# PJLab-ADG/nr3d_lib

Hardware: AMD Instinct MI355X
Metric: Mpoints/s LoTD fwd+bwd (16-lvl hash) + Mrays/s march+composite, 1 & 8 GPU (higher is better)
Workload: dtype f32; 1 GPU; configs[1]: 16-level Hash LoTD (gen_ngp_cfg: T=2^19, F=2, 6 Dense + 10 Hash), 2^20 points/GPU, fwd(+dy/dx) + dL/dx + dL/dparam, fp32; points_per_gpu=1048576, n_params=12131648, parallelism=single GPU

## Files before the change

nr3d_lib_amd/csrc/lotd_pair.hip:

```cpp
#include "lotd_device.h"
#include <stdlib.h>


namespace nr3d {
namespace lotd {

constexpr uint32_t kPEpbMax = 8192;
constexpr int kPAccThreads = 1024;
constexpr int kPLdsMax = 2 * (int)kPEpbMax;
constexpr int kPMaxLv = 32;
constexpr uint32_t kPMaxNb = 511;
typedef uint32_t u32x4 __attribute__((ext_vector_type(4)));

struct PairPlan {
	uint32_t qmap[kPMaxLv];
	uint32_t nb[kPMaxLv];
	uint32_t epb[kPMaxLv];
	uint32_t shift[kPMaxLv];
	uint32_t bucket_base[kPMaxLv + 1];
	uint32_t offs_base[kPMaxLv];
	uint32_t n_blk, n_pseudo;
	uint32_t cap;
	uint32_t lg;
	uint32_t sum_log2;
// ... 318 lines not shown
		uint32_t gbits;
		if constexpr (!SECOND) {
			gbits = max(__float_as_uint(g0) & 0x7FFFFFFFu, __float_as_uint(g1) & 0x7FFFFFFFu);
			if (ql == 0 && i < n)
				for (uint32_t e = 0; e < dp.n; ++e) {
					const uint32_t qd = dp.qmap[e];
					if ((int32_t)meta_level_of(md, qd) > max_level) continue;
					gbits = max(gbits, __float_as_uint(g[(int64_t)i * g_sn + (int64_t)(qd * 2) * g_se]) & 0x7FFFFFFFu);
					gbits = max(gbits, __float_as_uint(g[(int64_t)i * g_sn + (int64_t)(qd * 2 + 1) * g_se]) & 0x7FFFFFFFu);
				}
		} else {
			auto bound = [&](const Lvl &Lq, float ga, float gb) {
				const float m = __uint_as_float(max(__float_as_uint(ga) & 0x7FFFFFFFu, __float_as_uint(gb) & 0x7FFFFFFFu)) * 1.5f *
				                ((float)(Lq.res[0] - 2u) * fabsf(vin[0]) + (float)(Lq.res[1] - 2u) * fabsf(vin[1]) + (float)(Lq.res[2] - 2u) * fabsf(vin[2]));
				return __float_as_uint(m) & 0x7FFFFFFFu;
			};
			gbits = bound(L, g0, g1);
			if (ql == 0 && i < n) {
				if (!active) {
#pragma unroll
					for (int d = 0; d < 3; ++d) vin[d] = vin_[(size_t)i * 3 + d];
				}
				for (uint32_t e = 0; e < dp.n; ++e) {
					const uint32_t qd = dp.qmap[e];
					if ((int32_t)meta_level_of(md, qd) > max_level) continue;
					const Lvl Ld = load_level(md, meta_level_of(md, qd));
					gbits = max(gbits, bound(Ld, g[(int64_t)i * g_sn + (int64_t)(qd * 2) * g_se], g[(int64_t)i * g_sn + (int64_t)(qd * 2 + 1) * g_se]));
				}
			}
		}
		pair_gmax<kPBP>(gbits, scan_lds, gmax);
	}
}

__device__ __forceinline__ uint32_t gmax_slots(const uint32_t *__restrict__ slots, uint32_t n_slots, uint32_t *red) {
	uint32_t m = 0;
	for (uint32_t k = threadIdx.x; k < n_slots; k += 1024u) m = max(m, slots[k]);
#pragma unroll
	for (int off = 32; off >= 1; off >>= 1) m = max(m, (uint32_t)__shfl_xor((int)m, off, 64));
	__syncthreads();
	if ((threadIdx.x & 63u) == 0) red[threadIdx.x >> 6] = m;
	__syncthreads();
	m = 0;
#pragma unroll
	for (int k = 0; k < 16; ++k) m = max(m, red[k]);
	__syncthreads();
	return m;
}

__device__ __forceinline__ void pair_plan_block(const PairPlan &plan, const uint32_t *__restrict__ offs_g, uint32_t n_units,
                                                uint32_t *__restrict__ tot, uint32_t *__restrict__ rep,
                                                uint32_t *__restrict__ item_start, uint32_t *__restrict__ ticket, uint32_t bid,
                                                uint32_t nblk, const uint32_t *__restrict__ slots, uint32_t n_slots,
                                                uint32_t *__restrict__ gmax_out, bool empty_one) {
	__shared__ uint64_t red[16];
	__shared__ uint64_t carry_s;
	__shared__ uint32_t last_s;
	const uint32_t lane = threadIdx.x & 63, wave = threadIdx.x >> 6;
	const uint32_t NB = plan.bucket_base[plan.n_pseudo];
	{
		const uint32_t fb = bid * 16 + wave;
		if (fb < NB) {
			uint32_t q = 0;
			while (q + 1 < plan.n_pseudo && plan.bucket_base[q + 1] <= fb) ++q;
			const uint32_t *ob0 = offs_g + plan.offs_base[q] + (size_t)(fb - plan.bucket_base[q]) * plan.n_blk;
			const uint32_t *ob1 = ob0 + plan.n_blk;
			uint32_t sum = 0;
			for (uint32_t blk = lane; blk < plan.n_blk; blk += 64) sum += ob1[blk] - ob0[blk];
#pragma unroll
			for (int off = 32; off >= 1; off >>= 1) sum += __shfl_xor(sum, off, 64);
			if (lane == 0) __hip_atomic_store(tot + fb, sum, __ATOMIC_RELAXED, __HIP_MEMORY_SCOPE_AGENT);
		}
	}
	__syncthreads();
	if (threadIdx.x == 0) {
		__builtin_amdgcn_fence(__ATOMIC_RELEASE, "agent");
		asm volatile("s_waitcnt vmcnt(0)" ::: "memory");
		last_s = (atomicAdd(ticket, 1u) == nblk - 1u) ? 1u : 0u;
		__builtin_amdgcn_fence(__ATOMIC_ACQUIRE, "agent");
	}
	__syncthreads();
	if (!last_s) return;
	if (slots) {
		const uint32_t gb = gmax_slots(slots, n_slots, reinterpret_cast<uint32_t *>(red));
		if (threadIdx.x == 0) gmax_out[0] = gb;
	}
	auto ld_tot = [&](uint32_t fb) { return (uint64_t)__hip_atomic_load(tot + fb, __ATOMIC_RELAXED, __HIP_MEMORY_SCOPE_AGENT); };
	uint64_t part = 0;
	for (uint32_t fb = threadIdx.x; fb < NB; fb += 1024) part += ld_tot(fb);
#pragma unroll
	for (int off = 32; off >= 1; off >>= 1) part += __shfl_xor(part, off, 64);
	if (lane == 0) red[wave] = part;
	__syncthreads();
	uint64_t total = 0;
#pragma unroll
	for (int w = 0; w < 16; ++w) total += red[w];
	const uint64_t unit = total / n_units > 0 ? total / n_units : 1;
	if (threadIdx.x == 0) carry_s = 0;
	__syncthreads();
	for (uint32_t base = 0; base < NB; base += 1024) {
		const uint32_t fb = base + threadIdx.x;
		uint32_t r = 0;
		if (fb < NB) {
			const uint64_t t = ld_tot(fb);
			r = t == 0 ? (empty_one ? 1u : 0u) : (uint32_t)((t + unit / 2) / unit);
			if (t != 0 && r < 1) r = 1;
			if (r > plan.n_blk) r = plan.n_blk;
			rep[fb] = r;
		}
		uint64_t inc = r;
#pragma unroll
		for (int off = 1; off < 64; off <<= 1) { const uint64_t t2 = __shfl_up(inc, off, 64); if ((int)lane >= off) inc += t2; }
		__syncthreads();
		if (lane == 63) red[wave] = inc;
		__syncthreads();
		uint64_t woff = 0, tsum = 0;
#pragma unroll
		for (int w = 0; w < 16; ++w) { if (w < (int)wave) woff += red[w]; tsum += red[w]; }
		const uint64_t c = carry_s;
		if (fb < NB) item_start[fb] = (uint32_t)(c + woff + inc - r);
		__syncthreads();
		if (threadIdx.x == 0) carry_s = c + tsum;
		__syncthreads();
	}
	if (threadIdx.x == 0) item_start[NB] = (uint32_t)carry_s;
}
__global__ __launch_bounds__(1024) void k_pair_plan(PairPlan plan, const uint32_t *__restrict__ offs_g, uint32_t n_units,
                                                    uint32_t *__restrict__ tot, uint32_t *__restrict__ rep,
                                                    uint32_t *__restrict__ item_start, uint32_t *__restrict__ ticket,
                                                    const uint32_t *__restrict__ slots, uint32_t n_slots, uint32_t *__restrict__ gmax_out,
                                                    uint32_t empty_one) {
	pair_plan_block(plan, offs_g, n_units, tot, rep, item_start, ticket, blockIdx.x, gridDim.x, slots, n_slots, gmax_out, empty_one != 0u);
}

__device__ __forceinline__ float *pair_target(const Lvl &L, uint32_t epb, uint32_t lg, uint32_t foff0, uint32_t b, uint32_t t,
                                              float *__restrict__ dparam, bool out_half = false) {
	const uint32_t f = t >> lg, el = t & ((1u << lg) - 1u);
	const uint64_t entry = (uint64_t)b * epb + el;
	if (el >= epb || entry >= L.size) return nullptr;
	const uint64_t at = L.off + (entry * L.F + foff0 + f);
	return out_half ? reinterpret_cast<float *>(reinterpret_cast<__half *>(dparam) + at) : dparam + at;
}
__device__ __forceinline__ float pair_ld(const float *p, bool out_half) {
	return out_half ? __half2float(*reinterpret_cast<const __half *>(p)) : *p;
}
__device__ __forceinline__ void pair_st(float *p, float v, bool out_half) {
	if (out_half) *reinterpret_cast<__half *>(p) = __float2half(v); else *p = v;
}

struct PairFix { double scale, inv; bool on; };
__device__ __forceinline__ PairFix pair_fix_bits(uint32_t bits, uint32_t sum_log2) {
	PairFix f;
	f.on = bits < 0x7F800000u;
	const int e = max((int)(bits >> 23), 1) - 126;
	const int lim = min(62 - (int)sum_log2, 50 - 6);
	const int sc = max(min(lim - e, 1000), -1000);
	f.scale = __longlong_as_double((long long)(sc + 1023) << 52);
	f.inv = __longlong_as_double((long long)(1023 - sc) << 52);
	return f;
}
__device__ __forceinline__ PairFix pair_fix(const uint32_t *__restrict__ gmax, uint32_t sum_log2) {
	return pair_fix_bits(((cu32_t)gmax)[0], sum_log2);
}
__device__ __forceinline__ unsigned long long to_fix(float v, double scale) {
	const double t = __fma_rn((double)v, scale, 0x1.8p52);
	return (unsigned long long)(__double_as_longlong(t) - 0x4338000000000000LL);
}

__device__ __forceinline__ float pair_replica_sum(const float *__restrict__ part_t, uint32_t R, uint32_t kPLds) {
	float sum = 0.0f;
	uint32_t r0 = 0;
	for (; r0 + 8 <= R; r0 += 8) {
		float v[8];
#pragma unroll
		for (int j = 0; j < 8; ++j) v[j] = part_t[(size_t)(r0 + j) * kPLds];
#pragma unroll
		for (int j = 0; j < 8; ++j) sum += v[j];
	}
	for (; r0 < R; ++r0) sum += part_t[(size_t)r0 * kPLds];
	return sum;
}
__device__ __forceinline__ void pair_direct_sum(const DirectPlan &dp, const nr3d_lotd_meta_t *__restrict__ md,
                                                const float *__restrict__ dpart, float *__restrict__ dparam, uint32_t out_half,
                                                uint32_t fb, uint32_t t) {
	const bool half_out = (out_half & 1u) != 0, assign = (out_half & 2u) != 0;
	uint32_t e = 0;
	while (e + 1 < dp.n && dp.bucket_base[e + 1] <= fb) ++e;
	const uint32_t b = fb - dp.bucket_base[e], q = dp.qmap[e];
	const Lvl L = load_level(md, meta_level_of(md, q));
	const uint32_t foff0 = meta_cnt_of(md, q) * 2u, kPLds = 2u << dp.lg;
	if (t >= kPLds) return;
	float *p = pair_target(L, dp.epb[e], dp.lg, foff0, b, t, dparam, half_out);
	if (!p) return;
	const float sum = pair_replica_sum(dpart + (size_t)fb * dp.R * kPLds + t, dp.R, kPLds);
	pair_st(p, (assign ? 0.0f : pair_ld(p, half_out)) + sum, half_out);
}

template <int kUnroll, bool FIX>
__global__ __launch_bounds__(kPAccThreads, 8)  void k_pair_accum(PairPlan plan, const nr3d_lotd_meta_t *__restrict__ md,
                                                             const u32x4 *__restrict__ rec,
                                                             const uint32_t *__restrict__ offs_g,
                                                             const uint32_t *__restrict__ rep_g,
                                                             const uint32_t *__restrict__ item_start,
                                                             const uint32_t *__restrict__ gmax,
                                                             float *__restrict__ partial, float *__restrict__ dparam,
                                                             uint32_t out_half, uint32_t *__restrict__ bticket, uint32_t n_dred,
                                                             DirectPlan dp, const float *__restrict__ dpart) {
	extern __shared__ __attribute__((aligned(16))) unsigned long long acc_raw[];
	__shared__ uint32_t last_s;
	if (blockIdx.x < n_dred) {
		const uint32_t rows = (2u << dp.lg) / kPAccThreads;
		pair_direct_sum(dp, md, dpart, dparam, out_half, blockIdx.x / rows, (blockIdx.x % rows) * kPAccThreads + threadIdx.x);
		return;
	}
	const uint32_t item = blockIdx.x - n_dred;
	double *acc = reinterpret_cast<double *>(acc_raw);
	const uint32_t NB = plan.bucket_base[plan.n_pseudo];
	const cu32_t istart = (cu32_t)item_start, irep = (cu32_t)rep_g;
	if (item >= istart[NB]) return;
	uint32_t lo = 0, hi = NB;
	while (hi - lo > 1) { const uint32_t mid = (lo + hi) >> 1; if (istart[mid] <= item) lo = mid; else hi = mid; }
	const uint32_t fb = lo, R = irep[fb], r = item - istart[fb];
	uint32_t q = 0;
	while (q + 1 < plan.n_pseudo && plan.bucket_base[q + 1] <= fb) ++q;
	const uint32_t b = fb - plan.bucket_base[q];
	const uint32_t qg = plan.qmap[q];
	const Lvl L = load_level(md, meta_level_of(md, qg));
	const uint32_t foff0 = meta_cnt_of(md, qg) * 2u, epb = plan.epb[q];
	PairFix fx = {1.0, 1.0, false};
	if constexpr (FIX) fx = pair_fix(gmax, plan.sum_log2);
	const bool fix = FIX && fx.on;

	const uint32_t kPEpb = 1u << plan.lg, kPLds = 2u << plan.lg;
	for (uint32_t t = threadIdx.x; t < kPLds; t += kPAccThreads) acc_raw[t] = 0ull;
	__syncthreads();

	const uint32_t lane = threadIdx.x & 63, wave = threadIdx.x >> 6;
	constexpr uint32_t n_waves = kPAccThreads / 64;
	const uint32_t blk_lo = 0u, blk_hi = (plan.n_blk > r) ? (plan.n_blk - r + R - 1u) / R : 0u;
	const uint32_t *ob0 = offs_g + plan.offs_base[q] + (size_t)b * plan.n_blk;
	const uint32_t *ob1 = ob0 + plan.n_blk;
	const uint32_t kPCap = plan.cap;
	const u32x4 *rec_q = rec + (size_t)q * plan.n_blk * (size_t)kPCap;
	const uint32_t per_wave = (blk_hi - blk_lo + n_waves - 1) / n_waves;
	const uint32_t w_lo = min(blk_lo + wave * per_wave, blk_hi), w_hi = min(w_lo + per_wave, blk_hi);
	constexpr int kGroup = 8;
	for (uint32_t blk0 = w_lo; blk0 < w_hi; blk0 += 64) {
		const uint32_t mb = blk0 + lane;
		const uint32_t s_l = (mb < w_hi) ? ob0[r + R * mb] : 0u;
		const uint32_t e_l = (mb < w_hi) ? ob1[r + R * mb] : 0u;
		const uint32_t n_run = min(64u, w_hi - blk0);
		const u32x4 *rec_b = rec_q + (size_t)(r + R * blk0) * kPCap;
		for (uint32_t j0 = 0; j0 < n_run; j0 += kGroup) {
			uint32_t pre[kGroup + 1], rbase[kGroup];
			pre[0] = 0;
#pragma unroll
			for (int u = 0; u < kGroup; ++u) {
				const uint32_t j = min(j0 + (uint32_t)u, 63u);
				const uint32_t s_j = __builtin_amdgcn_readlane(s_l, j), e_j = __builtin_amdgcn_readlane(e_l, j);
				const uint32_t nrec = (j0 + (uint32_t)u < n_run) ? e_j - s_j : 0u;
				rbase[u] = s_j + j * R * kPCap - pre[u];
				pre[u + 1] = pre[u] + nrec;
			}
			const uint32_t total = pre[kGroup];
			for (uint32_t p0 = 0; p0 < total; p0 += 64u * kUnroll) {
				u32x4 rv[kUnroll];
#pragma unroll
				for (int v = 0; v < kUnroll; ++v) {
					const uint32_t pos = p0 + 64u * (uint32_t)v + lane;
					uint32_t at = rbase[0];
#pragma unroll
					for (int u = 1; u < kGroup; ++u) at = (pos >= pre[u]) ? rbase[u] : at;
					rv[v] = __builtin_nontemporal_load(rec_b + (size_t)(pos < total ? at + pos : rbase[0]));
				}
#pragma unroll
				for (int v = 0; v < kUnroll; ++v)
					if (p0 + 64u * (uint32_t)v + lane < total) {
						const uint32_t h = rv[v].x, fl = (h >> 26) & 7u;
						const uint32_t i0 = h & 8191u, i1 = (h >> 13) & 8191u;
						const float w = __uint_as_float(rv[v].y), a0 = __uint_as_float(rv[v].z), a1 = __uint_as_float(rv[v].w);
						if (fl == 4u) {
							const uint32_t wyq = (((h >> 13) & 8191u) << 8) | (rv[v].y >> 24) | ((h >> 29) << 21), wzq = rv[v].y & 0xFFFFFFu;
							const float wy = (float)wyq * (1.0f / 16777215.0f), wz = (float)wzq * (1.0f / 16777215.0f);
							const float q00 = (1.0f - wy) * (1.0f - wz), q01 = (1.0f - wy) * wz, q10 = wy * (1.0f - wz), q11 = wy * wz;
							const uint32_t i2 = i0 + L.res[2];
							if (fix) {
								atomicAdd(&acc_raw[i0], to_fix(q00 * a0, fx.scale)); atomicAdd(&acc_raw[kPEpb + i0], to_fix(q00 * a1, fx.scale));
								atomicAdd(&acc_raw[i0 + 1u], to_fix(q01 * a0, fx.scale)); atomicAdd(&acc_raw[kPEpb + i0 + 1u], to_fix(q01 * a1, fx.scale));
								atomicAdd(&acc_raw[i2], to_fix(q10 * a0, fx.scale)); atomicAdd(&acc_raw[kPEpb + i2], to_fix(q10 * a1, fx.scale));
								atomicAdd(&acc_raw[i2 + 1u], to_fix(q11 * a0, fx.scale)); atomicAdd(&acc_raw[kPEpb + i2 + 1u], to_fix(q11 * a1, fx.scale));
							} else {
								atomicAdd(&acc[i0], (double)(q00 * a0)); atomicAdd(&acc[kPEpb + i0], (double)(q00 * a1));
								atomicAdd(&acc[i0 + 1u], (double)(q01 * a0)); atomicAdd(&acc[kPEpb + i0 + 1u], (double)(q01 * a1));
								atomicAdd(&acc[i2], (double)(q10 * a0)); atomicAdd(&acc[kPEpb + i2], (double)(q10 * a1));
								atomicAdd(&acc[i2 + 1u], (double)(q11 * a0)); atomicAdd(&acc[kPEpb + i2 + 1u], (double)(q11 * a1));
							}
							continue;
						}
						const bool pair = fl == 3u;
						const float wl = pair ? 1.0f - w : 1.0f, wh = pair ? w : 1.0f;
						if (fix) {
							if (fl & 1u) { atomicAdd(&acc_raw[i0], to_fix(wl * a0, fx.scale)); atomicAdd(&acc_raw[kPEpb + i0], to_fix(wl * a1, fx.scale)); }
							if (fl & 2u) { atomicAdd(&acc_raw[i1], to_fix(wh * a0, fx.scale)); atomicAdd(&acc_raw[kPEpb + i1], to_fix(wh * a1, fx.scale)); }
						} else {
							if (fl & 1u) { atomicAdd(&acc[i0], (double)(wl * a0)); atomicAdd(&acc[kPEpb + i0], (double)(wl * a1)); }
							if (fl & 2u) { atomicAdd(&acc[i1], (double)(wh * a0)); atomicAdd(&acc[kPEpb + i1], (double)(wh * a1)); }
						}
					}
			}
		}
	}
	__syncthreads();

	auto value = [&](uint32_t t) -> float {
		return fix ? (float)((double)(long long)acc_raw[t] * fx.inv) : (float)acc[t];
	};
	if (R > 1) {
		float *mine = partial + (size_t)item * kPLds;
		for (uint32_t t = threadIdx.x; t < kPLds; t += kPAccThreads) mine[t] = value(t);
		if (!bticket) return;
		asm volatile("s_waitcnt vmcnt(0)" ::: "memory");
		__syncthreads();
		if (threadIdx.x == 0) {
			__builtin_amdgcn_fence(__ATOMIC_RELEASE, "agent");
			asm volatile("s_waitcnt vmcnt(0)" ::: "memory");
			last_s = (atomicAdd(bticket + fb, 1u) == R - 1u) ? 1u : 0u;
			__builtin_amdgcn_fence(__ATOMIC_ACQUIRE, "agent");
			asm volatile("s_waitcnt vmcnt(0)" ::: "memory");
		}
		__syncthreads();
		if (!last_s) return;
		const bool half_out = (out_half & 1u) != 0, assign = (out_half & 2u) != 0;
		const float *part0 = partial + (size_t)istart[fb] * kPLds;
		for (uint32_t t = threadIdx.x; t < kPLds; t += kPAccThreads) {
			float *p = pair_target(L, epb, plan.lg, foff0, b, t, dparam, half_out);
			if (!p) continue;
			const float sum = pair_replica_sum(part0 + t, R, kPLds);
			pair_st(p, (assign ? 0.0f : pair_ld(p, half_out)) + sum, half_out);
		}
		return;
	}
	constexpr int kFlush = 8;
	for (uint32_t tb = threadIdx.x; tb < kPLds; tb += kPAccThreads * kFlush) {
		float *p[kFlush];
		float v[kFlush], old[kFlush];
#pragma unroll
		for (int k = 0; k < kFlush; ++k) {
			const uint32_t t = tb + (uint32_t)k * kPAccThreads;
			p[k] = (t < kPLds) ? pair_target(L, epb, plan.lg, foff0, b, t, dparam, (out_half & 1u) != 0) : nullptr;
			v[k] = p[k] ? value(t) : 0.0f;
		}
		const bool half_out = (out_half & 1u) != 0, assign = (out_half & 2u) != 0;
#pragma unroll
		for (int k = 0; k < kFlush; ++k) old[k] = (p[k] && !assign) ? pair_ld(p[k], half_out) : 0.0f;
#pragma unroll
		for (int k = 0; k < kFlush; ++k) if (p[k]) pair_st(p[k], old[k] + v[k], half_out);
	}
}

template <bool FIX, bool SECOND = false>
__global__ __launch_bounds__(kPAccThreads, 8) void k_pair_direct(DirectPlan dp, const nr3d_lotd_meta_t *__restrict__ md, uint32_t n,
                                                                 int32_t max_level, uint32_t smooth, const float *__restrict__ x,
                                                                 const float *__restrict__ g, int64_t g_sn, int64_t g_se,
                                                                 const uint32_t *__restrict__ gmax, float *__restrict__ partial,
                                                                 const float *__restrict__ vin_, uint32_t plan_rows, PairPlan plan,
                                                                 const uint32_t *__restrict__ offs_g, uint32_t n_units,
                                                                 uint32_t *__restrict__ tot, uint32_t *__restrict__ rep,
                                                                 uint32_t *__restrict__ item_start, uint32_t *__restrict__ ticket,
                                                                 const uint32_t *__restrict__ slots, uint32_t n_slots,
                                                                 uint32_t *__restrict__ gmax_out, uint32_t empty_one) {
	extern __shared__ __attribute__((aligned(16))) unsigned long long acc_raw[];
	__shared__ uint32_t queue[kPAccThreads / 64][128];
	if (blockIdx.y >= gridDim.y - plan_rows) {
		const uint32_t bid = (blockIdx.y - (gridDim.y - plan_rows)) * gridDim.x + blockIdx.x, nblk = (plan.bucket_base[plan.n_pseudo] + 15u) / 16u;
		if (bid < nblk) pair_plan_block(plan, offs_g, n_units, tot, rep, item_start, ticket, bid, nblk, slots, n_slots, gmax_out, empty_one != 0u);
		return;
	}
	double *acc = reinterpret_cast<double *>(acc_raw);
	const uint32_t r = blockIdx.x, fb = blockIdx.y;
	uint32_t e = 0;
	while (e + 1 < dp.n && dp.bucket_base[e + 1] <= fb) ++e;
	const uint32_t b = fb - dp.bucket_base[e], q = dp.qmap[e];
	const uint32_t level = meta_level_of(md, q);
	const Lvl L = load_level(md, level);
	const uint32_t kPEpb = 1u << dp.lg, kPLds = 2u << dp.lg;
	PairFix fx = {1.0, 1.0, false};
	if constexpr (FIX) fx = slots ? pair_fix_bits(gmax_slots(slots, n_slots, &queue[0][0]), dp.sum_log2) : pair_fix(gmax, dp.sum_log2);
	const bool fix = FIX && fx.on;
	for (uint32_t t = threadIdx.x; t < kPLds; t += kPAccThreads) acc_raw[t] = 0ull;
	__syncthreads();
	if ((int32_t)level <= max_level) {
		const uint32_t p_lo = r * dp.pts_per_rep;
		auto process = [&](uint32_t i) {
			float xp[3];
#pragma unroll
			for (int d = 0; d < 3; ++d) xp[d] = x[(size_t)i * 3 + d];
			const float g0 = g[(int64_t)i * g_sn + (int64_t)(q * 2) * g_se], g1 = g[(int64_t)i * g_sn + (int64_t)(q * 2 + 1) * g_se];
			uint32_t hdr[4], bkt[4], cell[3];
			constexpr int kW = SECOND ? 3 : 0;
			float A[4][2], wp[SECOND ? 4 : 1], vin[3] = {0.0f, 0.0f, 0.0f};
			bool valid;
			if constexpr (SECOND) {
#pragma unroll
				for (int d = 0; d < 3; ++d) vin[d] = vin_[(size_t)i * 3 + d];
			}
			uint32_t qmask;
			float wy_unused;
			pair_records<SECOND>(L, dp.shift[e], dp.epb[e], dp.lg, xp, g0, g1, smooth != 0, hdr, bkt, A, wp, cell, dp.nb[e], valid, vin, qmask, wy_unused, false);
			float lo[4][2], hi[4][2];
#pragma unroll
			for (int m = 0; m < 4; ++m)
#pragma unroll
				for (int f = 0; f < 2; ++f) { lo[m][f] = (1.0f - wp[m & kW]) * A[m][f]; hi[m][f] = wp[m & kW] * A[m][f]; }
			bool rotate = false;
			{
				const uint32_t ln = threadIdx.x & 63u;
				auto prev = [](uint32_t v) { return (uint32_t)__builtin_amdgcn_update_dpp(0, (int)v, 0x138, 0xf, 0xf, false); };
				bool same = ln > 0;
#pragma unroll
				for (int d = 0; d < 3; ++d) same = same && (prev(cell[d]) == cell[d]);
				same = same && (prev(1u) != 0u);
				rotate = (uint32_t)__popcll(__ballot(same)) >= dp.merge_min;
			}
			if (!valid) return;
			if (rotate) {
				const uint32_t ln = threadIdx.x & 63u;
				const bool sw = (ln & 4u) != 0u, fs = (ln & 8u) != 0u;
#pragma unroll
// ... 181 lines not shown
			while ((2ull << sh) * L.res[2] <= kPEpb) ++sh;
			epb = (1u << sh) * L.res[2];
			nb = (uint32_t)((((uint64_t)L.res[0] * L.res[1]) + (1ull << sh) - 1) >> sh);
		} else {
			sh = plan.lg; epb = kPEpb;
			nb = L.size <= kPEpb ? 1u : (L.size >> plan.lg);
		}
		plan.qmap[nq] = q; plan.nb[nq] = nb; plan.epb[nq] = epb; plan.shift[nq] = sh;
		plan.bucket_base[nq] = nq ? plan.bucket_base[nq - 1] + plan.nb[nq - 1] : 0u;
		plan.offs_base[nq] = (uint32_t)base;
		base += (uint64_t)(nb + 1) * plan.n_blk;
		++nq;
	}
	plan.n_pseudo = nq;
	plan.bucket_base[nq] = nq ? plan.bucket_base[nq - 1] + plan.nb[nq - 1] : 0u;
	offs_words = base;
}

static bool pair_direct_enabled() { return opt::on(NR3D_OPT_PAIR_DIRECT); }
static uint64_t pair_direct_plan(const PairPlan &full, uint32_t n, DirectPlan &dp) {
	dp.n = 0; dp.lg = full.lg; dp.sum_log2 = full.sum_log2; dp.R = 1; dp.pts_per_rep = n;
	dp.merge_min = kDirectRotate;
	dp.bucket_base[0] = 0;
	if (!pair_direct_enabled()) return 0;
	uint64_t mask = 0;
	for (uint32_t ql = 0; ql < full.n_pseudo && dp.n < kDirectMaxLv; ++ql) {
		if (full.nb[ql] > kDirectNb || full.qmap[ql] >= 64u) continue;
		if (dp.bucket_base[dp.n] + full.nb[ql] > kDirectMaxWg) break;
		const uint32_t e = dp.n++;
		dp.qmap[e] = full.qmap[ql]; dp.nb[e] = full.nb[ql]; dp.epb[e] = full.epb[ql]; dp.shift[e] = full.shift[ql];
		dp.bucket_base[e + 1] = dp.bucket_base[e] + full.nb[ql];
		mask |= 1ull << full.qmap[ql];
	}
	if (dp.n == 0 || dp.n == full.n_pseudo) { dp.n = 0; return 0; }
	const uint32_t nbk = dp.bucket_base[dp.n];
	uint32_t R = kDirectMaxWg / nbk;
	R = R > 128u ? 128u : R;
	const uint32_t by_points = div_up(n, 2048u);
	R = R > by_points ? by_points : R;
	dp.R = R < 1u ? 1u : R;
	dp.pts_per_rep = div_up(n, dp.R);
	return mask;
}

uint32_t pair_direct_levels(const nr3d_lotd_meta_t *m, uint32_t n_points) {
	PairPlan plan;
	uint64_t ow;
	pair_plan(m, n_points, 0, 0x7fffffff, plan, ow);
	DirectPlan dp;
	pair_direct_plan(plan, n_points, dp);
	return dp.n;
}

void pair_layout(const nr3d_lotd_meta_t *m, uint32_t n_chunk, uint64_t &rec_bytes, uint64_t &offs_bytes, uint64_t &plan_bytes,
                 uint64_t &part_bytes) {
	PairPlan plan;
	uint64_t ow;
	pair_plan(m, n_chunk, 0, 0x7fffffff, plan, ow);
	const uint32_t NB = plan.bucket_base[plan.n_pseudo];
	rec_bytes = (uint64_t)plan.n_pseudo * plan.n_blk * plan.cap * 16;
	offs_bytes = ((ow * 4 + 255) / 256) * 256;
	plan_bytes = (((uint64_t)NB * 3 + 4) * 4 + 255) / 256 * 256;
	part_bytes = (uint64_t)(kPairUnits + NB + kDirectMaxWg) * (2u << plan.lg) * 4;
}

void launch_plan_items(uint32_t NB, uint32_t n_blk, uint32_t units, const uint32_t *tot, uint32_t *rep, uint32_t *item_start,
                       hipStream_t st);

constexpr uint32_t kFoldHead = 64;
uint64_t pair_fold_layout(const nr3d_lotd_meta_t *m, uint32_t n, int32_t max_level, uint32_t &gcols, uint32_t &zero_words,
                          uint32_t &slot_off) {
	gcols = zero_words = slot_off = 0;
	if (!opt::on(NR3D_OPT_PAIR_FOLD) || !m || !pair_applies(m) || n == 0 || max_level < 0 || !dparam_one_pass(n)) return 0;
	if (2u * m->n_pseudo_levels != m->n_encoded_dims) return 0;
	uint32_t nq = 0;
	while (nq < m->n_pseudo_levels && (int32_t)m->map_levels[nq] <= max_level) ++nq;
	for (uint32_t q = nq; q < m->n_pseudo_levels; ++q)
		if ((int32_t)m->map_levels[q] <= max_level) return 0;
	if (nq == 0) return 0;
	PairPlan pl;
	uint64_t ow;
	pair_plan(m, n, 0, max_level, pl, ow);
	gcols = 2u * nq;
	zero_words = kFoldHead + pl.bucket_base[pl.n_pseudo];
	slot_off = (zero_words + 63u) & ~63u;
	return (uint64_t)(slot_off + div_up(n, (uint32_t)kBlock)) * 4u;
}

int pair_chunk(const DparamPass &p, DparamChunk &c) {
	const nr3d_lotd_meta_t *meta = p.meta, *md = p.meta_dev;
	const uint32_t n = c.n, units = kPairUnits;
	const uint32_t out_flags = (p.out_half ? 1u : 0u) | (p.assign ? 2u : 0u);
	const int32_t min_level = p.min_level, max_level = p.max_level;
	const float *x = c.xc, *g = c.gc, *vin = p.second ? c.vc : nullptr;
	const int64_t g_sn = c.sn, g_se = c.se;
	uint32_t *offs = c.offs, *plan_buf = c.plan_buf, *fold = p.fold;
	float *dparam = p.dparam, *partial = c.partial;
	hipStream_t st = p.st;
	uint32_t f_gcols = 0, f_zero = 0, f_slot = 0;
	if (fold && (vin || min_level > 0 || pair_fold_layout(meta, n, max_level, f_gcols, f_zero, f_slot) == 0)) fold = nullptr;
	const uint32_t *slots = fold ? fold + f_slot : nullptr;
	const uint32_t n_slots = div_up(n, (uint32_t)kBlock);
	PairPlan pl;
	uint64_t ow;
	pair_plan(meta, n, min_level, max_level, pl, ow);
	if (pl.n_pseudo == 0) return 0;
	DirectPlan dp;
	dp.n = 0;
	const uint32_t NB_full = pl.bucket_base[pl.n_pseudo];
	{
		const uint64_t skip = pair_direct_plan(pl, n, dp);
		if (skip) pair_plan(meta, n, min_level, max_level, pl, ow, skip);
	}
	uint32_t nb_max = 0;
	for (uint32_t q = 0; q < pl.n_pseudo; ++q) nb_max = nb_max > pl.nb[q] ? nb_max : pl.nb[q];
	const uint32_t NB = pl.bucket_base[pl.n_pseudo];
	uint32_t *tot = plan_buf, *rep = plan_buf + NB, *item_start = plan_buf + 2 * (size_t)NB;
	uint32_t *gmax = fold ? fold : plan_buf + 3 * (size_t)NB + 2;
	uint32_t *bticket = fold ? fold + kFoldHead : nullptr;
	const size_t bin_lds_max = (size_t)kPairBp * 4 * 16 + (size_t)(kPMaxNb + 2) * 8;
	static LdsOnce once_bin, once_acc;
	NR3D_TRY(NR3D_LDS_LIMIT(once_bin, c.dev, (int)bin_lds_max, k_pair_bin<kPairBp>, k_pair_bin<kPairBp, true>));
	NR3D_TRY(NR3D_LDS_LIMIT(once_acc, c.dev, kPLdsMax * 8, k_pair_direct<true>, k_pair_direct<false>, k_pair_direct<true, true>,
	                        k_pair_direct<false, true>, k_pair_accum<kPairUnroll, false>, k_pair_accum<kPairUnroll, true>));
	if (!fold) NR3D_HIP_CHECK(hipMemsetAsync(gmax, 0, 2 * sizeof(uint32_t), st));
	const size_t bin_lds = (size_t)kPairBp * 4 * 16 + (size_t)(nb_max + 1) * 4;
	const uint32_t quad_on = (!vin && pair_quad_enabled()) ? 1u : 0u;
#define NR3D_PAIR_BIN(BP) if (vin) NR3D_PAIR_BIN_(BP, true); else NR3D_PAIR_BIN_(BP, false)
#define NR3D_PAIR_BIN_(BP, SEC) hipLaunchKernelGGL((k_pair_bin<BP, SEC>), dim3(pl.n_blk, pl.n_pseudo), dim3(BP), bin_lds, st, pl, md, n, max_level, \
	meta->interpolation_type, x, g, g_sn, g_se, (u32x4 *)c.rec, offs, fold ? nullptr : gmax, dp, vin, quad_on)
	{
		prof::Scope ps(NR3D_PROF_LOTD_BIN, st);
		NR3D_PAIR_BIN(kPairBp);
	}
#undef NR3D_PAIR_BIN
#undef NR3D_PAIR_BIN_
	float *dpart = partial + (size_t)(units + NB_full) * (2u << pl.lg);
	const uint32_t nbk_direct = dp.n ? dp.bucket_base[dp.n] : 0u;
	const bool plan_in_direct = fold && dp.n && pl.n_pseudo;
	const uint32_t plan_rows = plan_in_direct ? div_up(div_up(NB, 16u), dp.R) : 0u;
	const uint32_t empty_one = (fold && (out_flags & 2u)) ? 1u : 0u;
	if (dp.n) {
		prof::Scope ps(NR3D_PROF_LOTD_DIRECT, st);
		auto direct = [&](auto kern) {
			hipLaunchKernelGGL(kern, dim3(dp.R, nbk_direct + plan_rows), dim3(kPAccThreads), (size_t)(16u << pl.lg), st, dp, md, n, max_level,
			                   meta->interpolation_type, x, g, g_sn, g_se, gmax, dpart, vin, plan_rows, pl, offs, units, tot, rep, item_start,
			                   gmax + 1, slots, n_slots, fold, empty_one);
		};
		if (vin) { if (pair_fixed()) direct(k_pair_direct<true, true>); else direct(k_pair_direct<false, true>); }
		else     { if (pair_fixed()) direct(k_pair_direct<true, false>); else direct(k_pair_direct<false, false>); }
	}
	if (pl.n_pseudo == 0) {
		if (dp.n)
			hipLaunchKernelGGL(k_pair_direct_reduce, dim3(nbk_direct, (2u << pl.lg) / kPAccThreads), dim3(kPAccThreads), 0, st, dp, md, dpart,
			                   dparam, out_flags);
		NR3D_LAUNCH_CHECK();
		return 0;
	}
	if (!plan_in_direct)
		hipLaunchKernelGGL(k_pair_plan, dim3(div_up(NB, 16)), dim3(1024), 0, st, pl, offs, units, tot, rep, item_start, gmax + 1, slots, n_slots,
		                   fold, empty_one);
	const uint32_t n_dred = fold ? nbk_direct * ((2u << pl.lg) / kPAccThreads) : 0u;
#define NR3D_PAIR_ACC(U, F) hipLaunchKernelGGL((k_pair_accum<U, F>), dim3(n_dred + units + NB), dim3(kPAccThreads), (size_t)(16u << pl.lg), st, pl, md, \
	(const u32x4 *)c.rec, offs, rep, item_start, gmax, partial, dparam, out_flags, bticket, n_dred, dp, dpart)
	{
		prof::Scope ps(NR3D_PROF_LOTD_ACCUM, st);
		if (pair_fixed()) NR3D_PAIR_ACC(kPairUnroll, true); else NR3D_PAIR_ACC(kPairUnroll, false);
	}
#undef NR3D_PAIR_ACC
	if (!fold)
		hipLaunchKernelGGL(k_pair_reduce, dim3(NB + nbk_direct * kRedRows, div_up((2u << pl.lg) / kPAccThreads, kRedRows)), dim3(kPAccThreads), 0, st, pl, md, rep,
		                   item_start, partial, dparam, out_flags, NB, dp, dpart);
	NR3D_LAUNCH_CHECK();
	return 0;
}

}
}
```

Baseline: 1150 Mpoints/s.

## Make pair accumulate kernel persistent with precomputed item table and prefetch

The plan kernel now writes a per-item descriptor table (bucket, pseudo-level, replica index, replica count), so accumulate workgroups no longer binary-search item_start. The accumulate kernel becomes persistent: the grid is capped at twice the CU count and each workgroup loops over items with a stride. It prefetches the next item's descriptor and first block bounds before flushing the current one, and clears LDS during the flush. This removes the per-item launch and setup cost and hides some latency. The trade-offs are fewer resident workgroups, which can cause load imbalance, an extra barrier per item, and a larger plan buffer.

```diff
diff --git a/nr3d_lib_amd/csrc/lotd_pair.hip b/nr3d_lib_amd/csrc/lotd_pair.hip
--- a/nr3d_lib_amd/csrc/lotd_pair.hip
+++ b/nr3d_lib_amd/csrc/lotd_pair.hip
@@ -394,7 +394,7 @@
                                                 uint32_t *__restrict__ tot, uint32_t *__restrict__ rep,
                                                 uint32_t *__restrict__ item_start, uint32_t *__restrict__ ticket, uint32_t bid,
                                                 uint32_t nblk, const uint32_t *__restrict__ slots, uint32_t n_slots,
-                                                uint32_t *__restrict__ gmax_out, bool empty_one) {
+                                                uint32_t *__restrict__ gmax_out, bool empty_one, u32x4 *__restrict__ items) {
 	__shared__ uint64_t red[16];
 	__shared__ uint64_t carry_s;
 	__shared__ uint32_t last_s;
@@ -460,7 +460,14 @@
 #pragma unroll
 		for (int w = 0; w < 16; ++w) { if (w < (int)wave) woff += red[w]; tsum += red[w]; }
 		const uint64_t c = carry_s;
-		if (fb < NB) item_start[fb] = (uint32_t)(c + woff + inc - r);
+		if (fb < NB) {
+			const uint32_t first = (uint32_t)(c + woff + inc - r);
+			item_start[fb] = first;
+			uint32_t q = 0;
+			while (q + 1 < plan.n_pseudo && plan.bucket_base[q + 1] <= fb) ++q;
+			const uint32_t qb = q | ((fb - plan.bucket_base[q]) << 8);
+			for (uint32_t k = 0; k < r && first + k < n_units + NB; ++k) items[first + k] = u32x4{fb, qb, k, r};
+		}
 		__syncthreads();
 		if (threadIdx.x == 0) carry_s = c + tsum;
 		__syncthreads();
@@ -471,8 +478,8 @@
                                                     uint32_t *__restrict__ tot, uint32_t *__restrict__ rep,
                                                     uint32_t *__restrict__ item_start, uint32_t *__restrict__ ticket,
                                                     const uint32_t *__restrict__ slots, uint32_t n_slots, uint32_t *__restrict__ gmax_out,
-                                                    uint32_t empty_one) {
-	pair_plan_block(plan, offs_g, n_units, tot, rep, item_start, ticket, blockIdx.x, gridDim.x, slots, n_slots, gmax_out, empty_one != 0u);
+                                                    uint32_t empty_one, u32x4 *__restrict__ items) {
+	pair_plan_block(plan, offs_g, n_units, tot, rep, item_start, ticket, blockIdx.x, gridDim.x, slots, n_slots, gmax_out, empty_one != 0u, items);
 }
 
 __device__ __forceinline__ float *pair_target(const Lvl &L, uint32_t epb, uint32_t lg, uint32_t foff0, uint32_t b, uint32_t t,
@@ -538,11 +545,26 @@
 	pair_st(p, (assign ? 0.0f : pair_ld(p, half_out)) + sum, half_out);
 }
 
+struct PairItem { uint32_t fb, q, b, r, R; };
+__device__ __forceinline__ PairItem pair_item(const u32x4 *__restrict__ items, uint32_t item) {
+	const cu32_t w = (cu32_t)(items + item);
+	PairItem it;
+	it.fb = w[0]; it.q = w[1] & 255u; it.b = w[1] >> 8; it.r = w[2]; it.R = w[3];
+	return it;
+}
+__device__ __forceinline__ void pair_wave_share(uint32_t n_blk, uint32_t r, uint32_t R, uint32_t wave, uint32_t &w_lo, uint32_t &w_hi) {
+	constexpr uint32_t n_waves = kPAccThreads / 64;
+	const uint32_t blk_hi = (n_blk > r) ? (n_blk - r + R - 1u) / R : 0u;
+	const uint32_t per_wave = (blk_hi + n_waves - 1) / n_waves;
+	w_lo = min(wave * per_wave, blk_hi);
+	w_hi = min(w_lo + per_wave, blk_hi);
+}
+
 template <int kUnroll, bool FIX>
 __global__ __launch_bounds__(kPAccThreads, 8)  void k_pair_accum(PairPlan plan, const nr3d_lotd_meta_t *__restrict__ md,
                                                              const u32x4 *__restrict__ rec,
                                                              const uint32_t *__restrict__ offs_g,
-                                                             const uint32_t *__restrict__ rep_g,
+                                                             const u32x4 *__restrict__ items,
                                                              const uint32_t *__restrict__ item_start,
                                                              const uint32_t *__restrict__ gmax,
                                                              float *__restrict__ partial, float *__restrict__ dparam,
@@ -555,148 +577,169 @@
 		pair_direct_sum(dp, md, dpart, dparam, out_half, blockIdx.x / rows, (blockIdx.x % rows) * kPAccThreads + threadIdx.x);
 		return;
 	}
-	const uint32_t item = blockIdx.x - n_dred;
+	const uint32_t G = gridDim.x - n_dred;
+	uint32_t item = blockIdx.x - n_dred;
 	double *acc = reinterpret_cast<double *>(acc_raw);
 	const uint32_t NB = plan.bucket_base[plan.n_pseudo];
-	const cu32_t istart = (cu32_t)item_start, irep = (cu32_t)rep_g;
-	if (item >= istart[NB]) return;
-	uint32_t lo = 0, hi = NB;
-	while (hi - lo > 1) { const uint32_t mid = (lo + hi) >> 1; if (istart[mid] <= item) lo = mid; else hi = mid; }
-	const uint32_t fb = lo, R = irep[fb], r = item - istart[fb];
-	uint32_t q = 0;
-	while (q + 1 < plan.n_pseudo && plan.bucket_base[q + 1] <= fb) ++q;
-	const uint32_t b = fb - plan.bucket_base[q];
-	const uint32_t qg = plan.qmap[q];
-	const Lvl L = load_level(md, meta_level_of(md, qg));
-	const uint32_t foff0 = meta_cnt_of(md, qg) * 2u, epb = plan.epb[q];
+	const uint32_t live = min(((cu32_t)item_start)[NB], kPairUnits + NB);
+	if (item >= live) return;
 	PairFix fx = {1.0, 1.0, false};
 	if constexpr (FIX) fx = pair_fix(gmax, plan.sum_log2);
 	const bool fix = FIX && fx.on;
+	const bool half_out = (out_half & 1u) != 0, assign = (out_half & 2u) != 0;
 
 	const uint32_t kPEpb = 1u << plan.lg, kPLds = 2u << plan.lg;
+	const uint32_t lane = threadIdx.x & 63, wave = (uint32_t)__builtin_amdgcn_readfirstlane((int)(threadIdx.x >> 6));
+	const uint32_t kPCap = plan.cap;
+	auto first_bounds = [&](const PairItem &it, uint32_t &s_l, uint32_t &e_l) {
+		uint32_t w_lo, w_hi;
+		pair_wave_share(plan.n_blk, it.r, it.R, wave, w_lo, w_hi);
+		const uint32_t *ob0 = offs_g + plan.offs_base[it.q] + (size_t)it.b * plan.n_blk;
+		const uint32_t mb = w_lo + lane;
+		const uint32_t at = it.r + it.R * (mb < w_hi ? mb : 0u);
+		const uint32_t s = ob0[at], e = ob0[plan.n_blk + at];
+		s_l = (mb < w_hi) ? s : 0u;
+		e_l = (mb < w_hi) ? e : 0u;
+	};
+	PairItem cur = pair_item(items, item);
+	uint32_t s_l, e_l;
+	first_bounds(cur, s_l, e_l);
 	for (uint32_t t = threadIdx.x; t < kPLds; t += kPAccThreads) acc_raw[t] = 0ull;
 	__syncthreads();
 
-	const uint32_t lane = threadIdx.x & 63, wave = threadIdx.x >> 6;
-	constexpr uint32_t n_waves = kPAccThreads / 64;
-	const uint32_t blk_lo = 0u, blk_hi = (plan.n_blk > r) ? (plan.n_blk - r + R - 1u) / R : 0u;
-	const uint32_t *ob0 = offs_g + plan.offs_base[q] + (size_t)b * plan.n_blk;
-	const uint32_t *ob1 = ob0 + plan.n_blk;
-	const uint32_t kPCap = plan.cap;
-	const u32x4 *rec_q = rec + (size_t)q * plan.n_blk * (size_t)kPCap;
-	const uint32_t per_wave = (blk_hi - blk_lo + n_waves - 1) / n_waves;
-	const uint32_t w_lo = min(blk_lo + wave * per_wave, blk_hi), w_hi = min(w_lo + per_wave, blk_hi);
-	constexpr int kGroup = 8;
-	for (uint32_t blk0 = w_lo; blk0 < w_hi; blk0 += 64) {
-		const uint32_t mb = blk0 + lane;
-		const uint32_t s_l = (mb < w_hi) ? ob0[r + R * mb] : 0u;
-		const uint32_t e_l = (mb < w_hi) ? ob1[r + R * mb] : 0u;
-		const uint32_t n_run = min(64u, w_hi - blk0);
-		const u32x4 *rec_b = rec_q + (size_t)(r + R * blk0) * kPCap;
-		for (uint32_t j0 = 0; j0 < n_run; j0 += kGroup) {
-			uint32_t pre[kGroup + 1], rbase[kGroup];
-			pre[0] = 0;
-#pragma unroll
-			for (int u = 0; u < kGroup; ++u) {
-				const uint32_t j = min(j0 + (uint32_t)u, 63u);
-				const uint32_t s_j = __builtin_amdgcn_readlane(s_l, j), e_j = __builtin_amdgcn_readlane(e_l, j);
-				const uint32_t nrec = (j0 + (uint32_t)u < n_run) ? e_j - s_j : 0u;
-				rbase[u] = s_j + j * R * kPCap - pre[u];
-				pre[u + 1] = pre[u] + nrec;
-			}
-			const uint32_t total = pre[kGroup];
-			for (uint32_t p0 = 0; p0 < total; p0 += 64u * kUnroll) {
-				u32x4 rv[kUnroll];
-#pragma unroll
-				for (int v = 0; v < kUnroll; ++v) {
-					const uint32_t pos = p0 + 64u * (uint32_t)v + lane;
-					uint32_t at = rbase[0];
-#pragma unroll
-					for (int u = 1; u < kGroup; ++u) at = (pos >= pre[u]) ? rbase[u] : at;
-					rv[v] = __builtin_nontemporal_load(rec_b + (size_t)(pos < total ? at + pos : rbase[0]));
-				}
-#pragma unroll
-				for (int v = 0; v < kUnroll; ++v)
-					if (p0 + 64u * (uint32_t)v + lane < total) {
-						const uint32_t h = rv[v].x, fl = (h >> 26) & 7u;
-						const uint32_t i0 = h & 8191u, i1 = (h >> 13) & 8191u;
-						const float w = __uint_as_float(rv[v].y), a0 = __uint_as_float(rv[v].z), a1 = __uint_as_float(rv[v].w);
-						if (fl == 4u) {
-							const uint32_t wyq = (((h >> 13) & 8191u) << 8) | (rv[v].y >> 24) | ((h >> 29) << 21), wzq = rv[v].y & 0xFFFFFFu;
-							const float wy = (float)wyq * (1.0f / 16777215.0f), wz = (float)wzq * (1.0f / 16777215.0f);
-							const float q00 = (1.0f - wy) * (1.0f - wz), q01 = (1.0f - wy) * wz, q10 = wy * (1.0f - wz), q11 = wy * wz;
-							const uint32_t i2 = i0 + L.res[2];
+	for (;;) {
+		const bool more = item + G < live;
+		const PairItem nxt = pair_item(items, more ? item + G : item);
+		const uint32_t fb = cur.fb, q = cur.q, b = cur.b, r = cur.r, R = cur.R;
+		const uint32_t qg = plan.qmap[q];
+		const Lvl L = load_level(md, meta_level_of(md, qg));
+		const uint32_t foff0 = meta_cnt_of(md, qg) * 2u, epb = plan.epb[q];
+		const uint32_t *ob0 = offs_g + plan.offs_base[q] + (size_t)b * plan.n_blk;
+		const uint32_t *ob1 = ob0 + plan.n_blk;
+		const u32x4 *rec_q = rec + (size_t)q * plan.n_blk * (size_t)kPCap;
+		uint32_t w_lo, w_hi;
+		pair_wave_share(plan.n_blk, r, R, wave, w_lo, w_hi);
+		constexpr int kGroup = 8;
+		for (uint32_t blk0 = w_lo; blk0 < w_hi; blk0 += 64) {
+			if (blk0 != w_lo) {
+				const uint32_t mb = blk0 + lane;
+				s_l = (mb < w_hi) ? ob0[r + R * mb] : 0u;
+				e_l = (mb < w_hi) ? ob1[r + R * mb] : 0u;
+			}
+			const uint32_t n_run = min(64u, w_hi - blk0);
+			const u32x4 *rec_b = rec_q + (size_t)(r + R * blk0) * kPCap;
+			for (uint32_t j0 = 0; j0 < n_run; j0 += kGroup) {
+				uint32_t pre[kGroup + 1], rbase[kGroup];
+				pre[0] = 0;
+#pragma unroll
+				for (int u = 0; u < kGroup; ++u) {
+					const uint32_t j = min(j0 + (uint32_t)u, 63u);
+					const uint32_t s_j = __builtin_amdgcn_readlane(s_l, j), e_j = __builtin_amdgcn_readlane(e_l, j);
+					const uint32_t nrec = (j0 + (uint32_t)u < n_run) ? e_j - s_j : 0u;
+					rbase[u] = s_j + j * R * kPCap - pre[u];
+					pre[u + 1] = pre[u] + nrec;
+				}
+				const uint32_t total = pre[kGroup];
+				for (uint32_t p0 = 0; p0 < total; p0 += 64u * kUnroll) {
+					u32x4 rv[kUnroll];
+#pragma unroll
+					for (int v = 0; v < kUnroll; ++v) {
+						const uint32_t pos = p0 + 64u * (uint32_t)v + lane;
+						uint32_t at = rbase[0];
+#pragma unroll
+						for (int u = 1; u < kGroup; ++u) at = (pos >= pre[u]) ? rbase[u] : at;
+						rv[v] = __builtin_nontemporal_load(rec_b + (size_t)(pos < total ? at + pos : rbase[0]));
+					}
+#pragma unroll
+					for (int v = 0; v < kUnroll; ++v)
+						if (p0 + 64u * (uint32_t)v + lane < total) {
+							const uint32_t h = rv[v].x, fl = (h >> 26) & 7u;
+							const uint32_t i0 = h & 8191u, i1 = (h >> 13) & 8191u;
+							const float w = __uint_as_float(rv[v].y), a0 = __uint_as_float(rv[v].z), a1 = __uint_as_float(rv[v].w);
+							if (fl == 4u) {
+								const uint32_t wyq = (((h >> 13) & 8191u) << 8) | (rv[v].y >> 24) | ((h >> 29) << 21), wzq = rv[v].y & 0xFFFFFFu;
+								const float wy = (float)wyq * (1.0f / 16777215.0f), wz = (float)wzq * (1.0f / 16777215.0f);
+								const float q00 = (1.0f - wy) * (1.0f - wz), q01 = (1.0f - wy) * wz, q10 = wy * (1.0f - wz), q11 = wy * wz;
+								const uint32_t i2 = i0 + L.res[2];
+								if (fix) {
+									atomicAdd(&acc_raw[i0], to_fix(q00 * a0, fx.scale)); atomicAdd(&acc_raw[kPEpb + i0], to_fix(q00 * a1, fx.scale));
+									atomicAdd(&acc_raw[i0 + 1u], to_fix(q01 * a0, fx.scale)); atomicAdd(&acc_raw[kPEpb + i0 + 1u], to_fix(q01 * a1, fx.scale));
+									atomicAdd(&acc_raw[i2], to_fix(q10 * a0, fx.scale)); atomicAdd(&acc_raw[kPEpb + i2], to_fix(q10 * a1, fx.scale));
+									atomicAdd(&acc_raw[i2 + 1u], to_fix(q11 * a0, fx.scale)); atomicAdd(&acc_raw[kPEpb + i2 + 1u], to_fix(q11 * a1, fx.scale));
+								} else {
+									atomicAdd(&acc[i0], (double)(q00 * a0)); atomicAdd(&acc[kPEpb + i0], (double)(q00 * a1));
+									atomicAdd(&acc[i0 + 1u], (double)(q01 * a0)); atomicAdd(&acc[kPEpb + i0 + 1u], (double)(q01 * a1));
+									atomicAdd(&acc[i2], (double)(q10 * a0)); atomicAdd(&acc[kPEpb + i2], (double)(q10 * a1));
+									atomicAdd(&acc[i2 + 1u], (double)(q11 * a0)); atomicAdd(&acc[kPEpb + i2 + 1u], (double)(q11 * a1));
+								}
+								continue;
+							}
+							const bool pair = fl == 3u;
+							const float wl = pair ? 1.0f - w : 1.0f, wh = pair ? w : 1.0f;
 							if (fix) {
-								atomicAdd(&acc_raw[i0], to_fix(q00 * a0, fx.scale)); atomicAdd(&acc_raw[kPEpb + i0], to_fix(q00 * a1, fx.scale));
-								atomicAdd(&acc_raw[i0 + 1u], to_fix(q01 * a0, fx.scale)); atomicAdd(&acc_raw[kPEpb + i0 + 1u], to_fix(q01 * a1, fx.scale));
-								atomicAdd(&acc_raw[i2], to_fix(q10 * a0, fx.scale)); atomicAdd(&acc_raw[kPEpb + i2], to_fix(q10 * a1, fx.scale));
-								atomicAdd(&acc_raw[i2 + 1u], to_fix(q11 * a0, fx.scale)); atomicAdd(&acc_raw[kPEpb + i2 + 1u], to_fix(q11 * a1, fx.scale));
+								if (fl & 1u) { atomicAdd(&acc_raw[i0], to_fix(wl * a0, fx.scale)); atomicAdd(&acc_raw[kPEpb + i0], to_fix(wl * a1, fx.scale)); }
+								if (fl & 2u) { atomicAdd(&acc_raw[i1], to_fix(wh * a0, fx.scale)); atomicAdd(&acc_raw[kPEpb + i1], to_fix(wh * a1, fx.scale)); }
 							} else {
-								atomicAdd(&acc[i0], (double)(q00 * a0)); atomicAdd(&acc[kPEpb + i0], (double)(q00 * a1));
-								atomicAdd(&acc[i0 + 1u], (double)(q01 * a0)); atomicAdd(&acc[kPEpb + i0 + 1u], (double)(q01 * a1));
-								atomicAdd(&acc[i2], (double)(q10 * a0)); atomicAdd(&acc[kPEpb + i2], (double)(q10 * a1));
-								atomicAdd(&acc[i2 + 1u], (double)(q11 * a0)); atomicAdd(&acc[kPEpb + i2 + 1u], (double)(q11 * a1));
+								if (fl & 1u) { atomicAdd(&acc[i0], (double)(wl * a0)); atomicAdd(&acc[kPEpb + i0], (double)(wl * a1)); }
+								if (fl & 2u) { atomicAdd(&acc[i1], (double)(wh * a0)); atomicAdd(&acc[kPEpb + i1], (double)(wh * a1)); }
 							}
-							continue;
 						}
-						const bool pair = fl == 3u;
-						const float wl = pair ? 1.0f - w : 1.0f, wh = pair ? w : 1.0f;
-						if (fix) {
-							if (fl & 1u) { atomicAdd(&acc_raw[i0], to_fix(wl * a0, fx.scale)); atomicAdd(&acc_raw[kPEpb + i0], to_fix(wl * a1, fx.scale)); }
-							if (fl & 2u) { atomicAdd(&acc_raw[i1], to_fix(wh * a0, fx.scale)); atomicAdd(&acc_raw[kPEpb + i1], to_fix(wh * a1, fx.scale)); }
-						} else {
-							if (fl & 1u) { atomicAdd(&acc[i0], (double)(wl * a0)); atomicAdd(&acc[kPEpb + i0], (double)(wl * a1)); }
-							if (fl & 2u) { atomicAdd(&acc[i1], (double)(wh * a0)); atomicAdd(&acc[kPEpb + i1], (double)(wh * a1)); }
-						}
+				}
+			}
+		}
+		first_bounds(nxt, s_l, e_l);
+		__syncthreads();
+
+		auto take = [&](uint32_t t) -> float {
+			const float v = fix ? (float)((double)(long long)acc_raw[t] * fx.inv) : (float)acc[t];
+			acc_raw[t] = 0ull;
+			return v;
+		};
+		if (R > 1) {
+			float *mine = partial + (size_t)item * kPLds;
+			for (uint32_t t = threadIdx.x; t < kPLds; t += kPAccThreads) mine[t] = take(t);
+			if (bticket) {
+				asm volatile("s_waitcnt vmcnt(0)" ::: "memory");
+				__syncthreads();
+				if (threadIdx.x == 0) {
+					__builtin_amdgcn_fence(__ATOMIC_RELEASE, "agent");
+					asm volatile("s_waitcnt vmcnt(0)" ::: "memory");
+					last_s = (atomicAdd(bticket + fb, 1u) == R - 1u) ? 1u : 0u;
+					__builtin_amdgcn_fence(__ATOMIC_ACQUIRE, "agent");
+					asm volatile("s_waitcnt vmcnt(0)" ::: "memory");
+				}
+				__syncthreads();
+				if (last_s) {
+					const float *part0 = partial + (size_t)(item - r) * kPLds;
+					for (uint32_t t = threadIdx.x; t < kPLds; t += kPAccThreads) {
+						float *p = pair_target(L, epb, plan.lg, foff0, b, t, dparam, half_out);
+						if (!p) continue;
+						const float sum = pair_replica_sum(part0 + t, R, kPLds);
+						pair_st(p, (assign ? 0.0f : pair_ld(p, half_out)) + sum, half_out);
 					}
-			}
-		}
-	}
-	__syncthreads();
-
-	auto value = [&](uint32_t t) -> float {
-		return fix ? (float)((double)(long long)acc_raw[t] * fx.inv) : (float)acc[t];
-	};
-	if (R > 1) {
-		float *mine = partial + (size_t)item * kPLds;
-		for (uint32_t t = threadIdx.x; t < kPLds; t += kPAccThreads) mine[t] = value(t);
-		if (!bticket) return;
-		asm volatile("s_waitcnt vmcnt(0)" ::: "memory");
+				}
+			}
+		} else {
+			constexpr int kFlush = 8;
+			for (uint32_t tb = threadIdx.x; tb < kPLds; tb += kPAccThreads * kFlush) {
+				float *p[kFlush];
+				float v[kFlush], old[kFlush];
+#pragma unroll
+				for (int k = 0; k < kFlush; ++k) {
+					const uint32_t t = tb + (uint32_t)k * kPAccThreads;
+					p[k] = (t < kPLds) ? pair_target(L, epb, plan.lg, foff0, b, t, dparam, half_out) : nullptr;
+					v[k] = (t < kPLds) ? take(t) : 0.0f;
+				}
+#pragma unroll
+				for (int k = 0; k < kFlush; ++k) old[k] = (p[k] && !assign) ? pair_ld(p[k], half_out) : 0.0f;
+#pragma unroll
+				for (int k = 0; k < kFlush; ++k) if (p[k]) pair_st(p[k], old[k] + v[k], half_out);
+			}
+		}
+		if (!more) return;
 		__syncthreads();
-		if (threadIdx.x == 0) {
-			__builtin_amdgcn_fence(__ATOMIC_RELEASE, "agent");
-			asm volatile("s_waitcnt vmcnt(0)" ::: "memory");
-			last_s = (atomicAdd(bticket + fb, 1u) == R - 1u) ? 1u : 0u;
-			__builtin_amdgcn_fence(__ATOMIC_ACQUIRE, "agent");
-			asm volatile("s_waitcnt vmcnt(0)" ::: "memory");
-		}
-		__syncthreads();
-		if (!last_s) return;
-		const bool half_out = (out_half & 1u) != 0, assign = (out_half & 2u) != 0;
-		const float *part0 = partial + (size_t)istart[fb] * kPLds;
-		for (uint32_t t = threadIdx.x; t < kPLds; t += kPAccThreads) {
-			float *p = pair_target(L, epb, plan.lg, foff0, b, t, dparam, half_out);
-			if (!p) continue;
-			const float sum = pair_replica_sum(part0 + t, R, kPLds);
-			pair_st(p, (assign ? 0.0f : pair_ld(p, half_out)) + sum, half_out);
-		}
-		return;
-	}
-	constexpr int kFlush = 8;
-	for (uint32_t tb = threadIdx.x; tb < kPLds; tb += kPAccThreads * kFlush) {
-		float *p[kFlush];
-		float v[kFlush], old[kFlush];
-#pragma unroll
-		for (int k = 0; k < kFlush; ++k) {
-			const uint32_t t = tb + (uint32_t)k * kPAccThreads;
-			p[k] = (t < kPLds) ? pair_target(L, epb, plan.lg, foff0, b, t, dparam, (out_half & 1u) != 0) : nullptr;
-			v[k] = p[k] ? value(t) : 0.0f;
-		}
-		const bool half_out = (out_half & 1u) != 0, assign = (out_half & 2u) != 0;
-#pragma unroll
-		for (int k = 0; k < kFlush; ++k) old[k] = (p[k] && !assign) ? pair_ld(p[k], half_out) : 0.0f;
-#pragma unroll
-		for (int k = 0; k < kFlush; ++k) if (p[k]) pair_st(p[k], old[k] + v[k], half_out);
+		item += G;
+		cur = nxt;
 	}
 }
 
@@ -710,12 +753,13 @@
                                                                  uint32_t *__restrict__ tot, uint32_t *__restrict__ rep,
                                                                  uint32_t *__restrict__ item_start, uint32_t *__restrict__ ticket,
                                                                  const uint32_t *__restrict__ slots, uint32_t n_slots,
-                                                                 uint32_t *__restrict__ gmax_out, uint32_t empty_one) {
+                                                                 uint32_t *__restrict__ gmax_out, uint32_t empty_one,
+                                                                 u32x4 *__restrict__ items) {
 	extern __shared__ __attribute__((aligned(16))) unsigned long long acc_raw[];
 	__shared__ uint32_t queue[kPAccThreads / 64][128];
 	if (blockIdx.y >= gridDim.y - plan_rows) {
 		const uint32_t bid = (blockIdx.y - (gridDim.y - plan_rows)) * gridDim.x + blockIdx.x, nblk = (plan.bucket_base[plan.n_pseudo] + 15u) / 16u;
-		if (bid < nblk) pair_plan_block(plan, offs_g, n_units, tot, rep, item_start, ticket, bid, nblk, slots, n_slots, gmax_out, empty_one != 0u);
+		if (bid < nblk) pair_plan_block(plan, offs_g, n_units, tot, rep, item_start, ticket, bid, nblk, slots, n_slots, gmax_out, empty_one != 0u, items);
 		return;
 	}
 	double *acc = reinterpret_cast<double *>(acc_raw);
@@ -1003,6 +1047,21 @@
 	return dp.n;
 }
 
+static uint64_t pair_items_offset(uint32_t NB) { return (((uint64_t)NB * 3 + 4) * 4 + 255) / 256 * 64; }
+
+static int pair_resident_wgs(int dev, uint32_t &n) {
+	static std::atomic<uint32_t> cached[64];
+	uint32_t v = (dev >= 0 && dev < 64) ? cached[dev].load(std::memory_order_relaxed) : 0u;
+	if (v == 0) {
+		int cus = 0;
+		NR3D_HIP_CHECK(hipDeviceGetAttribute(&cus, hipDeviceAttributeMultiprocessorCount, dev));
+		v = 2u * (uint32_t)(cus > 0 ? cus : 1);
+		if (dev >= 0 && dev < 64) cached[dev].store(v, std::memory_order_relaxed);
+	}
+	n = v;
+	return 0;
+}
+
 void pair_layout(const nr3d_lotd_meta_t *m, uint32_t n_chunk, uint64_t &rec_bytes, uint64_t &offs_bytes, uint64_t &plan_bytes,
                  uint64_t &part_bytes) {
 	PairPlan plan;
@@ -1011,7 +1070,7 @@
 	const uint32_t NB = plan.bucket_base[plan.n_pseudo];
 	rec_bytes = (uint64_t)plan.n_pseudo * plan.n_blk * plan.cap * 16;
 	offs_bytes = ((ow * 4 + 255) / 256) * 256;
-	plan_bytes = (((uint64_t)NB * 3 + 4) * 4 + 255) / 256 * 256;
+	plan_bytes = pair_items_offset(NB) * 4 + ((uint64_t)(kPairUnits + NB) * 16 + 255) / 256 * 256;
 	part_bytes = (uint64_t)(kPairUnits + NB + kDirectMaxWg) * (2u << plan.lg) * 4;
 }
 
@@ -1067,6 +1126,7 @@
 	for (uint32_t q = 0; q < pl.n_pseudo; ++q) nb_max = nb_max > pl.nb[q] ? nb_max : pl.nb[q];
 	const uint32_t NB = pl.bucket_base[pl.n_pseudo];
 	uint32_t *tot = plan_buf, *rep = plan_buf + NB, *item_start = plan_buf + 2 * (size_t)NB;
+	u32x4 *items = (u32x4 *)(plan_buf + pair_items_offset(NB));
 	uint32_t *gmax = fold ? fold : plan_buf + 3 * (size_t)NB + 2;
 	uint32_t *bticket = fold ? fold + kFoldHead : nullptr;
 	const size_t bin_lds_max = (size_t)kPairBp * 4 * 16 + (size_t)(kPMaxNb + 2) * 8;
@@ -1096,7 +1156,7 @@
 		auto direct = [&](auto kern) {
 			hipLaunchKernelGGL(kern, dim3(dp.R, nbk_direct + plan_rows), dim3(kPAccThreads), (size_t)(16u << pl.lg), st, dp, md, n, max_level,
 			                   meta->interpolation_type, x, g, g_sn, g_se, gmax, dpart, vin, plan_rows, pl, offs, units, tot, rep, item_start,
-			                   gmax + 1, slots, n_slots, fold, empty_one);
+			                   gmax + 1, slots, n_slots, fold, empty_one, items);
 		};
 		if (vin) { if (pair_fixed()) direct(k_pair_direct<true, true>); else direct(k_pair_direct<false, true>); }
 		else     { if (pair_fixed()) direct(k_pair_direct<true, false>); else direct(k_pair_direct<false, false>); }
@@ -1110,10 +1170,13 @@
 	}
 	if (!plan_in_direct)
 		hipLaunchKernelGGL(k_pair_plan, dim3(div_up(NB, 16)), dim3(1024), 0, st, pl, offs, units, tot, rep, item_start, gmax + 1, slots, n_slots,
-		                   fold, empty_one);
+		                   fold, empty_one, items);
 	const uint32_t n_dred = fold ? nbk_direct * ((2u << pl.lg) / kPAccThreads) : 0u;
-#define NR3D_PAIR_ACC(U, F) hipLaunchKernelGGL((k_pair_accum<U, F>), dim3(n_dred + units + NB), dim3(kPAccThreads), (size_t)(16u << pl.lg), st, pl, md, \
-	(const u32x4 *)c.rec, offs, rep, item_start, gmax, partial, dparam, out_flags, bticket, n_dred, dp, dpart)
+	uint32_t n_res = 0;
+	NR3D_TRY(pair_resident_wgs(c.dev, n_res));
+	const uint32_t n_accum = n_res < units + NB ? n_res : units + NB;
+#define NR3D_PAIR_ACC(U, F) hipLaunchKernelGGL((k_pair_accum<U, F>), dim3(n_dred + n_accum), dim3(kPAccThreads), (size_t)(16u << pl.lg), st, pl, md, \
+	(const u32x4 *)c.rec, offs, items, item_start, gmax, partial, dparam, out_flags, bticket, n_dred, dp, dpart)
 	{
 		prof::Scope ps(NR3D_PROF_LOTD_ACCUM, st);
 		if (pair_fixed()) NR3D_PAIR_ACC(kPairUnroll, true); else NR3D_PAIR_ACC(kPairUnroll, false);
```

New measurement: 1128 Mpoints/s. 0.981x the previous value.
